# juhyeonkim95/Mitsuba3DopplerToF

Measured on AMD Instinct MI355X. Metric: Mpaths/s (whole node), Doppler Cornell 512x512 64spp, higher is better.
Workload: dtype f32

## Files before the change

### include/dtof.h

```cpp
#ifndef DTOF_H
#define DTOF_H
#include <stdint.h>
#include <stddef.h>

#ifdef __cplusplus
extern "C" {
#endif

#define DTOF_OK            0
#define DTOF_ERR_INVALID   1
#define DTOF_ERR_HIP       2
#define DTOF_ERR_CANCELLED 3

typedef struct dtof_scene   dtof_scene;
typedef struct dtof_sampler dtof_sampler;

const char *dtof_version(void);
const char *dtof_last_error(void);

int dtof_scene_load_file(const char *path, const char *const *param_names, const char *const *param_values,
                         int n_params, dtof_scene **out);
int dtof_scene_load_string(const char *xml, const char *const *param_names, const char *const *param_values,
                           int n_params, dtof_scene **out);
void dtof_scene_destroy(dtof_scene *scene);
// ... 147 lines not shown
int  dtof_sampler_seed(dtof_sampler *s, uint32_t seed, uint32_t wavefront_size);
int  dtof_sampler_set_samples_per_wavefront(dtof_sampler *s, uint32_t spw);
int  dtof_sampler_advance(dtof_sampler *s);
int  dtof_sampler_next_1d(dtof_sampler *s, float *out);
int  dtof_sampler_next_2d(dtof_sampler *s, float *out_xy);
int  dtof_sampler_next_1d_correlate(dtof_sampler *s, const uint8_t *correlate, int correlate_all, float *out);
int  dtof_sampler_next_2d_correlate(dtof_sampler *s, const uint8_t *correlate, int correlate_all, float *out_xy);
int  dtof_sampler_next_1d_time(dtof_sampler *s, int strategy, float antithetic_shift, int stratify_each_interval, float *out);
int  dtof_sampler_get_state(dtof_sampler *s, uint32_t *out7);
int  dtof_sampler_fork(const dtof_sampler *s, dtof_sampler **out);
int  dtof_sampler_clone(const dtof_sampler *s, dtof_sampler **out);
int  dtof_sampler_set_sample_count(dtof_sampler *s, uint32_t sample_count);
int  dtof_sampler_seeded(const dtof_sampler *s);
uint32_t dtof_sampler_wavefront_size(const dtof_sampler *s);
uint32_t dtof_sampler_sample_count(const dtof_sampler *s);

int dtof_eval_modulation(dtof_scene *scene, int mode, const float *t, const float *len, float *out, uint32_t n);

int dtof_ray_intersect(dtof_scene *scene, uint32_t n, const float *rays8, float *out19, int32_t *ids3);
int dtof_ray_intersect_uv(dtof_scene *scene, uint32_t n, const float *rays8, float *out19, int32_t *ids3, float *uv4);
int dtof_ray_test(dtof_scene *scene, uint32_t n, const float *rays8, int32_t *occluded);
int dtof_flat_query(dtof_scene *scene, int form, int any, uint32_t n, const float *rays8, float *out3, int32_t *ids);
int dtof_flat_query_pairs(dtof_scene *scene, int any, uint32_t n, const float *rays8, float *out3, int32_t *ids);
int dtof_tree_query(dtof_scene *scene, int form, int any, uint32_t n, const float *rays8, float *out3, int32_t *ids3);

#define DTOF_COMP_MICROFACET_EVAL          0
#define DTOF_COMP_MICROFACET_PDF           1
#define DTOF_COMP_MICROFACET_G1            2
#define DTOF_COMP_MICROFACET_SAMPLE        3
#define DTOF_COMP_FRESNEL                  4
#define DTOF_COMP_FRESNEL_CONDUCTOR        5
#define DTOF_COMP_RFILTER                  6
#define DTOF_COMP_WARP_COSINE_HEMISPHERE   7
#define DTOF_COMP_WARP_DISK_CONCENTRIC     8
#define DTOF_COMP_WARP_UNIFORM_TRIANGLE    9
#define DTOF_COMP_WARP_UNIFORM_SPHERE     10
#define DTOF_COMP_COORDINATE_SYSTEM       11
#define DTOF_COMP_TEA_FLOAT32             12
#define DTOF_COMP_MATH                    13
int dtof_eval_component(int component, const float *params, int n_params, const float *in, int in_stride, float *out, int out_stride, uint32_t n);

#ifdef __cplusplus
}
#endif
#endif
```

### mitsuba3dopplertof_amd/__init__.py

```python
import ctypes as C
import os

import numpy as np

__all__ = ["load_file", "load_string", "load_dict", "Scene", "Integrator", "Sampler", "DtofError", "render",
           "render_multi_pass", "to_tof_image", "lib_path", "ETimeSampling", "velocity_map_variants", "MOMENT_PLANES", "aov_channels", "AOV_TYPES"]

_HERE = os.path.dirname(os.path.abspath(__file__))
_LIB = None


class DtofError(RuntimeError):
    pass


class ETimeSampling:
    UNIFORM, STRATIFIED, ANTITHETIC, ANTITHETIC_MIRROR, PERIODIC, REGULAR = 0, 1, 2, 3, 4, 5


class _Stats(C.Structure):
    _fields_ = [("n_paths", C.c_uint64), ("n_bounces", C.c_uint64), ("n_shadow_rays", C.c_uint64),
                ("ms_total", C.c_double), ("ms_generate", C.c_double), ("ms_trace", C.c_double),
                ("ms_shade", C.c_double), ("ms_shadow", C.c_double), ("ms_splat", C.c_double),
                ("n_launches_trace", C.c_uint32), ("n_launches_shade", C.c_uint32), ("n_launches_shadow", C.c_uint32),
# ... 98 lines not shown
    L.dtof_eval_component.argtypes = [C.c_int, vp, C.c_int, vp, C.c_int, vp, C.c_int, C.c_uint32]
    L.dtof_render_rows_async.argtypes = [vp, C.c_uint32, C.c_uint32, C.c_int32, C.c_int32, vp, C.c_int, vp]
    L.dtof_clear_async.argtypes = [vp, vp, C.c_size_t]
    L.dtof_camera_rays.argtypes = [vp, C.c_uint32, vp, vp]
    L.dtof_bsdf_eval.argtypes = [vp, C.c_uint32, C.c_uint32, vp, vp]
    L.dtof_bsdf_eval_ex.argtypes = [vp, C.c_uint32, C.c_int, C.c_uint32, vp, vp]
    L.dtof_scene_set_stream.argtypes = [vp, vp]
    L.dtof_scene_set_film_layout.argtypes = [vp, C.c_int32, C.c_uint64]
    L.dtof_render_stripes_async.argtypes = [vp, C.c_uint32, C.c_uint32, C.c_int32, C.c_int32, C.c_int32, vp, C.c_int, vp]
    L.dtof_develop_async.argtypes = [vp, vp, vp, C.c_int64]
    L.dtof_async_collect.argtypes = [vp, vp, vp, C.c_uint32, vp]
    L.dtof_ray_intersect.argtypes = [vp, C.c_uint32, vp, vp, vp]
    L.dtof_ray_intersect_uv.argtypes = [vp, C.c_uint32, vp, vp, vp, vp]
    L.dtof_ray_test.argtypes = [vp, C.c_uint32, vp, vp]
    rows, stripes = [vp, C.c_uint32, C.c_uint32, C.c_int32, C.c_int32, vp, C.c_int, vp], [vp, C.c_uint32, C.c_uint32, C.c_int32, C.c_int32, C.c_int32, vp, C.c_int, vp]
    for name, args in (("dtof_render_variants", [vp, C.c_uint32, C.c_uint32, vp, C.c_int, vp, C.POINTER(_Stats)]),
                       ("dtof_render_rows_variants", rows + [C.POINTER(_Stats)]), ("dtof_render_rows_variants_async", rows),
                       ("dtof_render_stripes_variants", stripes + [C.POINTER(_Stats)]), ("dtof_render_stripes_variants_async", stripes),
                       ("dtof_sample_lanes_variants", [vp, C.c_uint32, C.c_uint32, vp, C.c_int, C.c_uint64, C.c_uint64, vp, vp, vp]),
                       ("dtof_emitter_eval", [vp, C.c_int, C.c_int, C.c_int32, C.c_uint32, vp, vp]),
                       ("dtof_flat_query", [vp, C.c_int, C.c_int, C.c_uint32, vp, vp, vp]),
                       ("dtof_flat_query_pairs", [vp, C.c_int, C.c_uint32, vp, vp, vp]),
                       ("dtof_tree_query", [vp, C.c_int, C.c_int, C.c_uint32, vp, vp, vp]),
                       ("dtof_develop_accumulate_async", [vp, vp, C.c_int32, C.c_uint64, vp, C.c_int64, C.c_int]),
                       ("dtof_velocity_map_async", [vp, vp, C.c_int, vp, vp, C.c_uint32, C.c_double, C.c_double, C.c_int64, vp, vp, vp]),
                       ("dtof_velocity_map_variants", [vp, C.c_int, vp]),
                       ("dtof_render_velocity_map", [vp, C.c_uint32, C.c_uint32, vp, C.c_int, C.c_double, C.c_double, vp, vp, vp, C.POINTER(_Stats)]),
                       ("dtof_render_velocity_map_f64", [vp, C.c_uint32, C.c_uint32, vp, C.c_int, C.c_double, C.c_double, vp, vp, vp, C.POINTER(_Stats)]),
                       ("dtof_render_variants_f64", [vp, C.c_uint32, C.c_uint32, vp, C.c_int, vp, vp, C.POINTER(_Stats)]),
                       ("dtof_render_rows_variants_f64", rows[:-1] + [vp, C.c_int32, C.c_uint64, C.POINTER(_Stats)]),
                       ("dtof_develop_f64_async", [vp, vp, vp, C.c_int64]), ("dtof_develop_rgba_f64_async", [vp, vp, vp, vp, C.c_int64]),
                       ("dtof_moment_planes", [C.c_int]),
                       ("dtof_render_moments", [vp, C.c_uint32, C.c_uint32, C.c_uint32, vp, C.c_int, C.c_int, vp, C.POINTER(_Stats)]),
                       ("dtof_aov_parse", [C.c_char_p, vp, C.c_int, C.POINTER(C.c_int), vp, C.c_size_t, C.POINTER(C.c_int)]),
                       ("dtof_scene_get_aovs", [vp, vp, C.c_size_t]),
                       ("dtof_render_aovs", [vp, C.c_uint32, C.c_uint32, C.c_uint32, vp, C.c_int, C.c_int, vp, C.POINTER(_Stats)]),
                       ("dtof_sample_aov_lanes", [vp, C.c_uint32, C.c_uint32, vp, C.c_int, C.c_uint64, C.c_uint64, vp, vp])):
        if hasattr(L, name):
            getattr(L, name).argtypes = args
    _LIB = L
    return L


FLAT_GEOMETRY = np.array([[1, 0, 0,  0, 1, 0,  0, 0, 1,  1, 0, 0,  0, 1, 0,  0, 0, 1]], np.float32)


# ... 443 lines not shown
                "wi": out[:, 16:19], "ids": ids, "uv": uv[:, 0:2], "prim_uv": uv[:, 2:4], "prim_index": ids[:, 2], "valid": ids[:, 0] >= 0}

    def ray_test(self, o, d, time=0.0, maxt=None):
        rays = self._rays(o, d, time, maxt)
        occ = np.zeros(len(rays), np.int32)
        _check(_lib().dtof_ray_test(self._h, len(rays), rays.ctypes.data, occ.ctypes.data))
        return occ != 0

    FLAT_FORMS = {"generic": 0, "one_wall": 1, "shape": 2}

    def flat_query(self, rays8, form=0, any=False):
        rays = np.ascontiguousarray(rays8, np.float32).reshape(-1, 8)
        form = self.FLAT_FORMS.get(form, form)
        out, ids = np.zeros((len(rays), 3), np.float32), np.zeros(len(rays), np.int32)
        _check(_lib().dtof_flat_query(self._h, int(form), 1 if any else 0, len(rays), rays.ctypes.data, None if any else out.ctypes.data, ids.ctypes.data))
        return ids if any else {"t": out[:, 0], "u": out[:, 1], "v": out[:, 2], "obj": ids}

    def flat_query_pairs(self, rays8, any=False):
        rays = np.ascontiguousarray(rays8, np.float32).reshape(-1, 8)
        out, ids = np.zeros((len(rays), 3), np.float32), np.zeros(len(rays), np.int32)
        _check(_lib().dtof_flat_query_pairs(self._h, 1 if any else 0, len(rays), rays.ctypes.data, None if any else out.ctypes.data, ids.ctypes.data))
        return ids if any else {"t": out[:, 0], "u": out[:, 1], "v": out[:, 2], "obj": ids}

    TREE_FORMS = {"float": 0, "half_overflow": 1, "half_overflow_tlas_lds": 2, "defer_pair": 3, "half_every_shape": 4}

    def tree_query(self, rays8, form=0, any=False):
        rays = np.ascontiguousarray(rays8, np.float32).reshape(-1, 8)
        form = self.TREE_FORMS.get(form, form)
        out, ids = np.zeros((len(rays), 3), np.float32), np.zeros(len(rays) if any else (len(rays), 3), np.int32)
        _check(_lib().dtof_tree_query(self._h, int(form), 1 if any else 0, len(rays), rays.ctypes.data, None if any else out.ctypes.data, ids.ctypes.data))
        return ids if any else {"t": out[:, 0], "u": out[:, 1], "v": out[:, 2], "ids": ids}

    def cancel(self):
        _lib().dtof_cancel(self._h)


COMPONENTS = {"microfacet_eval": (0, 1), "microfacet_pdf": (1, 1), "microfacet_g1": (2, 1), "microfacet_sample": (3, 4), "fresnel": (4, 4),
              "fresnel_conductor": (5, 1), "rfilter": (6, 1), "warp_cosine_hemisphere": (7, 3), "warp_disk_concentric": (8, 2),
              "warp_uniform_triangle": (9, 2), "warp_uniform_sphere": (10, 3), "coordinate_system": (11, 6), "tea_float32": (12, 1), "math": (13, 1)}


def eval_component(name, inputs, params=()):
    comp, n_out = COMPONENTS[name]
    x = np.ascontiguousarray(np.atleast_2d(np.asarray(inputs, np.float32)))
    p = np.ascontiguousarray(np.asarray(params, np.float32).reshape(-1))
    out = np.zeros((len(x), n_out), np.float32)
# ... 183 lines not shown
```

### mitsuba3dopplertof_amd/csrc/dtof_kernels.h

```cpp
#pragma once
#include <stdint.h>
#include <hip/hip_runtime.h>
#include "dtof_math.h"

namespace dtof {

constexpr uint32_t kChunkBlocks = 8;
constexpr uint32_t kMaxInline = 4;
constexpr int kMaxOffsets = 4;

struct RenderParams {
    float s2c[16];
    float cam_to_world[12];
    float near_clip, far_clip, shutter_open, shutter_open_time;
    int32_t orthographic;
    float aperture_radius, focus_distance;
    int32_t crop_x, crop_y, crop_w, crop_h;
    float scale_x, scale_y, offset_x, offset_y;
    int32_t filter; float filter_radius, inv_radius;
    float gauss_coeff[10];
    float filter_b, filter_c;
    uint32_t base_seed, seed, seed_value;
    uint32_t spp, spp_log2;
    uint32_t tcn, pcn;
// ... 149 lines not shown
constexpr uint32_t kHeadlineC2Facts = (DTOF_HEADLINE_C2) != 0 && kHeadlineFusedFacts != 0 ? (kHeadlineFusedFacts | (DTOF_HEADLINE_C2)) : 0u;
static_assert(((DTOF_HEADLINE_C2) & ~kFactsSampling) == 0, "DTOF_HEADLINE_C2 names route facts only (bits 13 and up)");
#ifndef DTOF_HEADLINE_SHAPE_COUNT
#define DTOF_HEADLINE_SHAPE_COUNT 5
#endif
#ifndef DTOF_HEADLINE_SHAPE_WALL
#define DTOF_HEADLINE_SHAPE_WALL 2
#endif
constexpr uint32_t kHeadlineShapeFacts = (DTOF_HEADLINE_SHAPE_COUNT) != 0 && (kHeadlineC2Facts & kFactOneWall) != 0 ? (kHeadlineC2Facts | flat_shape_fact(DTOF_HEADLINE_SHAPE_COUNT, DTOF_HEADLINE_SHAPE_WALL)) : 0u;
static_assert((DTOF_HEADLINE_SHAPE_COUNT) == 0 || (kHeadlineC2Facts & kFactOneWall) == 0 || (kHeadlineShapeFacts & kFactFlatShape) != 0, "a shape has 1 .. 8 objects and the wall among them");
#ifndef DTOF_HEADLINE_PAIR
#define DTOF_HEADLINE_PAIR 1
#endif
#ifndef DTOF_STREAM_JUMPS
#define DTOF_STREAM_JUMPS 1
#endif
#ifndef DTOF_PAIR_SAMPLES
#define DTOF_PAIR_SAMPLES 1
#endif
constexpr uint32_t kHeadlinePairFacts = DTOF_HEADLINE_PAIR && kHeadlineShapeFacts != 0 ? (kHeadlineShapeFacts | kFactPairSamples) : 0u;
#ifndef DTOF_PAIR_WALK_PRIMARY
#define DTOF_PAIR_WALK_PRIMARY 1
#endif
#ifdef DTOF_TRAVERSAL_STATS
constexpr bool kPairWalkCompiled = false;
#else
constexpr bool kPairWalkCompiled = true;
#endif
constexpr bool pair_walk_shape(uint32_t facts) { return (facts & kFactOneWall) != 0 && flat_shape_count(facts) == 5 && flat_shape_wall(facts) == 2; }
#ifndef DTOF_FLAT_SHAPE_ANY
#define DTOF_FLAT_SHAPE_ANY 1
#endif
#ifndef DTOF_FLAT_SHAPE_CLOSEST
#define DTOF_FLAT_SHAPE_CLOSEST 1
#endif
#ifndef DTOF_WALL_FRAMES
#define DTOF_WALL_FRAMES 1
#endif
#ifndef DTOF_RESIDENT_FACTS
#define DTOF_RESIDENT_FACTS 0x37f
#endif
constexpr uint32_t kResidentFacts = DTOF_RESIDENT_FACTS;

struct ShadeLaunch { bool staged; int mode; uint32_t waves, grid, lds, lds_flat; hipStream_t stream; ShadeArgs args; uint32_t facts; };
uint32_t launch_shade_plain(bool area, bool k4, const ShadeLaunch &L);
void launch_shade_mesh(bool area, bool k4, const ShadeLaunch &L);
// ... 77 lines not shown
```

### mitsuba3dopplertof_amd/csrc/dtof_render.hip

```cpp
#include "../../include/dtof.h"
#include "dtof_kernels.h"
#include "dtof_reconstruct.h"
#include "dtof_film64.h"
#include "dtof_moments.h"
#include "dtof_aov.h"
#include "dtof_flat_query.h"
#include "dtof_tree_query.h"
#include "dtof_scene.h"
#include "dtof_math.h"
#include <atomic>
#include <dlfcn.h>
#include <cstdio>
#include <cstring>
#include <cstdlib>
#include <cmath>
#include <string>
#include <memory>
#include <vector>

using namespace dtof;

namespace {

thread_local std::string g_last_error;

struct HipError : std::runtime_error { using std::runtime_error::runtime_error; };
#define HIP_CHECK(expr) do { hipError_t e_ = (expr); if (e_ != hipSuccess) \
    throw HipError(std::string(#expr) + ": " + hipGetErrorString(e_)); } while (0)

// ... 1800 lines not shown
        if (n & 1u) throw std::runtime_error("dtof_flat_query_pairs: an odd number of rays");
        if (n > (1u << 24)) throw std::runtime_error("dtof_flat_query_pairs: more than 2^24 rays in one call");
        for (uint32_t i = 0; i < n; i += 2) {
            const float *a = rays8 + (size_t) i * 8, *b = a + 8;
            if (memcmp(a, b, 24) != 0 || memcmp(a + 7, b + 7, 4) != 0)
                throw std::runtime_error("dtof_flat_query_pairs: rays " + std::to_string(i) + " and " + std::to_string(i + 1) + " differ in o, d or maxt");
        }
        const SceneTraits t = scene_traits(*sc);
        const FlatChoice c = flat_choice(t, t.blas_triangles <= 32768 && sc->host.textures.empty(), true, true);
        if (!kFlatQueryPairsBuilt || c.flat_objects == 0 || !(c.facts & kFactOneWall) || (c.facts & kFlatShapeFields) != (flat_query_facts(2) & kFlatShapeFields))
            throw std::runtime_error("dtof_flat_query_pairs: the pair form is compiled for a flat table of 5 rectangles whose one instance, of one rectangle, is at index 2" +
                                     (c.flat_objects ? ", this table has " + std::to_string(c.flat_objects) + " objects" : std::string(", this scene has no flat table")));
        ensure_device(sc);
        DevBuf<float> dr, dout; DevBuf<int32_t> dids;
        dr.ensure((size_t) n * 8); dout.ensure(any ? 1 : (size_t) n * 3); dids.ensure(n);
        if (n) HIP_CHECK(hipMemcpy(dr.p, rays8, (size_t) n * 32, hipMemcpyHostToDevice));
        launch_flat_query(sc->d_blob.p, (uint32_t) sc->blob.size(), t.flat_off, c.flat_objects, c.memo_obj, kFlatQueryPairs, any != 0, dr.p, dout.p, dids.p, n, nullptr);
        HIP_CHECK(hipGetLastError());
        if (n && !any) HIP_CHECK(hipMemcpy(out3, dout.p, (size_t) n * 12, hipMemcpyDeviceToHost));
        if (n) HIP_CHECK(hipMemcpy(ids, dids.p, (size_t) n * 4, hipMemcpyDeviceToHost));
    });
}

int dtof_tree_query(dtof_scene *sc, int form, int any, uint32_t n, const float *rays8, float *out3, int32_t *ids3) {
    return guarded([&] {
        if (!sc || (n && (!rays8 || !ids3 || (!any && !out3)))) throw std::runtime_error("null argument");
        if (n > (1u << 24)) throw std::runtime_error("dtof_tree_query: more than 2^24 rays in one call");
        const SceneTraits t = scene_traits(*sc);
        const TreeQueryScene q { t.stack_depth, t.n_tlas_nodes, t.has_nodes16, t.has_analytic };
        if (const char *why = tree_query_refusal(form, q)) throw std::runtime_error(std::string("dtof_tree_query: ") + why);
        ensure_device(sc);
        const size_t per = any ? 1 : 3;
        DevBuf<float> dr, dout; DevBuf<int32_t> dids;
        dr.ensure((size_t) n * 8); dout.ensure(any ? 1 : (size_t) n * 3); dids.ensure((size_t) n * per);
        if (n) HIP_CHECK(hipMemcpy(dr.p, rays8, (size_t) n * 32, hipMemcpyHostToDevice));
        launch_tree_query(sc->d_blob.p, q, form, any != 0, dr.p, dout.p, dids.p, n, nullptr);
        HIP_CHECK(hipGetLastError());
        if (n && !any) HIP_CHECK(hipMemcpy(out3, dout.p, (size_t) n * 12, hipMemcpyDeviceToHost));
        if (n) HIP_CHECK(hipMemcpy(ids3, dids.p, (size_t) n * per * 4, hipMemcpyDeviceToHost));
    });
}

#ifdef DTOF_TRAVERSAL_STATS
int dtof_debug_traversal_stats_n(unsigned long long *out8, uint32_t n) {
    return guarded([&] {
        HIP_CHECK(hipDeviceSynchronize());
// ... 10 lines not shown
```

### mitsuba3dopplertof_amd/csrc/dtof_sampling.h

```cpp
#pragma once
#include "dtof_kernels.h"
#include "dtof_scene.h"
#include "dtof_math.h"

#ifndef DTOF_D
#define DTOF_D __device__ __forceinline__
#endif

namespace dtof {

struct Rng { uint64_t state, inc; };
DTOF_D float next_f32(Rng &r) { return pcg_next_f32(r.state, r.inc); }
DTOF_D Rng seed_stream(uint32_t seed_value, uint32_t index) {
    uint32_t v0, v1; tea32(seed_value, index, v0, v1);
    Rng r; pcg_seed(v0, v1, r.state, r.inc); return r;
}
DTOF_D uint64_t stream_inc(uint32_t seed_value, uint32_t index) {
    uint32_t v0, v1; tea32(seed_value, index, v0, v1);
    return ((uint64_t) v1 << 1) | 1u;
}
DTOF_D float next_correlate(Rng &main, Rng &path, bool correlate) {
    uint64_t old = correlate ? path.state : main.state;
    path.state = path.state * kPcgMult + path.inc;
    main.state = main.state * kPcgMult + main.inc;
// ... 89 lines not shown
    V3 near_p = mk(r0 * iw, r1 * iw, r2 * iw);
    if (!PERSPECTIVE_ONLY && rp.orthographic) {
        o = xf_point(rp.cam_to_world, near_p);
        dw = normalize(xf_vector(rp.cam_to_world, mk(0.f, 0.f, 1.f)));
        maxt = rp.far_clip - rp.near_clip;
        return;
    }
    const bool lens = !PERSPECTIVE_ONLY && rp.aperture_radius != 0.f;
    V3 d;
    if (lens) {
        float tx, ty; concentric_disk(apx, apy, tx, ty);
        const V3 aperture_p = mk(rp.aperture_radius * tx, rp.aperture_radius * ty, 0.f);
        const float f_dist = rp.focus_distance / near_p.z;
        d = normalize(near_p * f_dist - aperture_p);
        o = xf_point(rp.cam_to_world, aperture_p);
    } else {
        d = normalize(near_p);
        o = mk(rp.cam_to_world[3], rp.cam_to_world[7], rp.cam_to_world[11]);
    }
    dw = xf_vector(rp.cam_to_world, d);
    float inv_z = rcp(d.z), near_t = rp.near_clip * inv_z, far_t = rp.far_clip * inv_z;
    o = o + dw * near_t;
    maxt = far_t - near_t;
}

template <bool PERSPECTIVE_ONLY = false, uint32_t FACTS = 0>
DTOF_D PrimaryLane generate_lane(const RenderParams &rp, uint32_t lane, bool wave_pixel = false, uint32_t vlane = 0) {
    constexpr bool F_SINGLE_PASS = (FACTS & kFactSinglePass) != 0, F_DOPPLER_CORR = (FACTS & kFactDopplerCorr) != 0, F_CORRELATED = (FACTS & kFactCorrelated) != 0;
    constexpr bool F_STRAT = (FACTS & kFactStratifiedPairs) != 0 && F_DOPPLER_CORR, F_SHIFTS = facts_lane_shifts(FACTS);
    const bool needs_tm = !F_STRAT && (F_DOPPLER_CORR || (rp.integrator == 0 && rp.sampler_kind == SAMPLER_CORRELATED)) && rp.time_sampling >= TIME_ANTITHETIC;
    Rng main, tm, path; tm.state = 0; tm.inc = 1;
    uint2 *const carried = !F_SINGLE_PASS && rp.n_passes > 1 ? rp.pass_rng + (size_t) (vlane - rp.pass_first) * 3 : nullptr;
    const uint32_t pass = F_SINGLE_PASS ? 0u : rp.pass;
    if (pass == 0 && wave_pixel && needs_tm && rp.tcn == 2 && rp.pcn == 2) {
        main = seed_stream(rp.seed_value, lane);
        const bool odd = lane & 1u;
        uint32_t a0, a1; tea32(rp.seed_value + (odd ? 2u : 1u), lane >> 1, a0, a1);
        const uint32_t b0 = (uint32_t) __builtin_amdgcn_update_dpp(0, (int) a0, 0xb1, 0xf, 0xf, false), b1 = (uint32_t) __builtin_amdgcn_update_dpp(0, (int) a1, 0xb1, 0xf, 0xf, false);
        pcg_seed(odd ? b0 : a0, odd ? b1 : a1, tm.state, tm.inc);
        pcg_seed(odd ? a0 : b0, odd ? a1 : b1, path.state, path.inc);
    } else if (pass == 0) {
        main = seed_stream(rp.seed_value, lane);
        if (needs_tm) tm = seed_stream(rp.seed_value + 1, fdiv(lane, rp.d_tcn));
        path = seed_stream(rp.seed_value + 2, F_STRAT ? lane >> 1 : fdiv(lane, rp.d_pcn));
    } else {
        const uint2 a = carried[0], b = carried[1], c = carried[2];
// ... 46 lines not shown
```

### mitsuba3dopplertof_amd/csrc/dtof_shade.h

```cpp
#pragma once
#include "dtof_device.h"
#include <atomic>
#include <initializer_list>
#include <type_traits>

namespace dtof {


DTOF_D uint32_t wave_append(bool pred, uint32_t &running) {
    const uint64_t mask = __ballot(pred);
    const uint32_t slot = running + (uint32_t) __popcll(mask & ((1ull << __lane_id()) - 1ull));
    running += (uint32_t) __popcll(mask);
    return slot;
}

struct BsdfOut { V3 val, weight, wo; float pdf, bs_pdf, bs_eta; bool bs_delta, bs_null; };
template <int SPEC, bool HAVE_WO = false>
DTOF_D void bsdf_eval_pdf_sample(const SceneView &sv, const DShape *sh, Surface &si, V3 wo, bool active_em, float sample_1, float s2x, float s2y, BsdfOut &out, bool want_sample = true, const V3 *diffuse_wo = nullptr) {
    const bool masked = SPEC && (sh->flags & SF_MASK);
    bool null_pick = false; float opacity = 1.f;
    if (masked) { opacity = mask_opacity_at(sv, sh, si.u, si.v); null_pick = !(sample_1 < opacity); sample_1 = sample_1 / opacity; }
    const bool blend = SPEC == 2 && (sh->flags & SF_BLEND);
    float blend_w = 0.f; bool pick_1 = false;
    if (blend) {
// ... 280 lines not shown
template <bool AREA, bool MESH, int SPEC, bool ONE_EMITTER = false>
void launch_emitter_eval_level(const uint8_t *scene, int mode, uint32_t index, float pmf, const float *in, float *out, uint32_t n, hipStream_t s) {
    if (n) hipLaunchKernelGGL((k_emitter_eval<AREA, MESH, SPEC, ONE_EMITTER>), dim3(nblk(n)), dim3(kBlock), 0, s, scene, mode, index, pmf, in, out, n);
}

template <bool LDS, int MODE, bool AREA, int KMAX, bool MESH, int SPEC, int RESW = 0, bool RH16 = false, uint32_t FACTS = 0>
#ifndef DTOF_MESH_WAVES
#define DTOF_MESH_WAVES 3
#endif
#ifndef DTOF_K4_RES_LDS
#define DTOF_K4_RES_LDS 1
#endif
__global__ __launch_bounds__(RESW ? RESW * 64 : kShadeBlock, RESW ? RESW / 4 : (MODE == 2 && !MESH && !SPEC && KMAX == 1) ? 4 : (MODE != 0 && MESH) ? ((SPEC && KMAX > 1) ? 2 : DTOF_MESH_WAVES) : 1) void k_shade(ShadeArgs args_by_value) {
    constexpr bool FUSED = MODE != 0, FIRST = MODE == 2;
    static_assert(FACTS == 0 || MODE == 2, "plan facts describe a first-bounce launch");
    constexpr bool F_SINGLE_PASS = (FACTS & kFactSinglePass) != 0, F_DOPPLER_CORR = (FACTS & kFactDopplerCorr) != 0, F_NO_LANE_OUT = (FACTS & kFactNoLaneOutput) != 0;
    constexpr bool F_IDENTITY = (FACTS & kFactIdentityQueue) != 0, F_NO_RR = (FACTS & kFactNoRoulette) != 0, F_CORRELATED = (FACTS & kFactCorrelated) != 0;
    constexpr bool F_WHOLE_PATH = (FACTS & kFactWholePath) != 0, F_ONE_BLOCK = (FACTS & kFactOneBlock) != 0, F_ONE_EMITTER = (FACTS & kFactOneEmitter) != 0;
    constexpr bool F_WAVE_PIXEL = (FACTS & kFactWavePixel) != 0;
    constexpr bool F_FLAT = (FACTS & kFactFlat) != 0, F_ONE_WALL = (FACTS & kFactOneWall) != 0, F_FUSED_SPLAT = (FACTS & kFactFusedSplat) != 0;
    constexpr bool F_EMITTER_SAMPLED = (FACTS & kFactEmitterSampled) != 0, F_ID24 = (FACTS & kFactIdShift24) != 0, F_SHIFTS = facts_lane_shifts(FACTS);
    constexpr bool F_PAIR = (FACTS & kFactPairSamples) != 0, JUMPS = F_PAIR && DTOF_STREAM_JUMPS, PAIR = F_PAIR && DTOF_PAIR_SAMPLES;
    constexpr bool WALK_PRIMARY = F_PAIR && DTOF_PAIR_WALK_PRIMARY && pair_walk_shape(FACTS);
    static_assert(!F_PAIR || F_WAVE_PIXEL, "a lane reads its partner's registers: the whole wave is active where it does");
    static_assert(!F_PAIR || (!AREA && SPEC == 0 && KMAX == 1 && F_ONE_EMITTER), "a diffuse BSDF picks no lobe and a lone point light samples nothing: of an iteration's six draws only s2x and s2y are read");
    static_assert(!F_PAIR || (F_NO_RR && F_CORRELATED && F_DOPPLER_CORR && F_WHOLE_PATH && F_SINGLE_PASS && (FACTS & kFactStratifiedPairs) != 0), "every draw comes from the stream lanes 2k and 2k + 1 share, none is looked at for roulette, no state outlives the launch");
    constexpr bool F_FRAMES = F_ONE_WALL && DTOF_WALL_FRAMES;
    static_assert(!F_FLAT || (!MESH && SPEC == 0 && RESW == 0), "trace_flat serves the staged rectangle-only diffuse kernels");
    static_assert(!F_ONE_WALL || F_FLAT, "the one wall is an object of the flat table");
    static_assert(!F_FUSED_SPLAT || KMAX == 1, "the fused splat is the one-film kernels'");
    static_assert(!F_WAVE_PIXEL || F_IDENTITY, "whole waves of one pixel are provable for an identity queue only");
    static_assert(!F_ONE_BLOCK || RESW == 0, "blocks per segment belong to the classic launch");
    constexpr bool RES_LDS = RESW != 0 && KMAX > 1 && DTOF_K4_RES_LDS;
    constexpr bool S16 = RESW != 0 && KMAX > 1;
    static_assert(!RES_LDS || 3 * KMAX == (int) kParkWords + 1, "the film-state columns hold all but the last float of the K results");
    constexpr bool PARK_ST = DTOF_PARK && RESW == 16 && KMAX == 1;
    constexpr bool PARK = DTOF_PARK && RESW == 16 && (KMAX == 1 || RES_LDS);
    constexpr uint32_t kRngAt = RES_LDS ? kParkWords : 0u;
    constexpr int KREG = RES_LDS ? 1 : KMAX;
    constexpr uint32_t kStackStride = RESW ? RESW * 64 : kShadeBlock;
    static_assert(RESW == 0 || (MODE == 2 && !LDS && MESH), "the resident stage exists for the unstaged fused first-bounce kernel with mesh code");
    static_assert(!RH16 || RESW != 0, "half-float LDS planes belong to the resident stage");
    extern __shared__ uint4 lds[];
    __shared__ uint32_t s_inline_all[(RESW ? RESW : 1) * 2 * kMaxInline];
    typedef const char __attribute__((address_space(4))) *KernargBytes;
    const KernargBytes kernarg = (KernargBytes) __builtin_amdgcn_kernarg_segment_ptr();
// ... 37 lines not shown
        sv_res.isect = (const DTriIsect *) (small + gh->off_isect);
        sv_res.emitters = (const DEmitter *) (small + gh->off_emitters);
    }
    for (;;) {
    uint32_t seg, sub_index = 0;
    if (RESW) {
        uint32_t taken = 0;
        if (lane_id == 0) taken = atomicAdd(A0.q.seg_counter, 1u);
        uint32_t unit = (uint32_t) __builtin_amdgcn_readfirstlane((int) taken);
        if (unit >= A0.n_seg * sub) break;
        unit = A0.n_seg * sub - 1u - unit;
        seg = sub > 1 ? unit / sub : unit; sub_index = sub > 1 ? unit - seg * sub : 0u;
    } else {
        seg = sub > 1 ? blockIdx.x / sub : blockIdx.x; sub_index = sub > 1 ? blockIdx.x - seg * sub : 0u;
    }
    const uint32_t count = seg_count(F_IDENTITY ? nullptr : A0.count_in, seg, A0.rp.n_lanes);
    uint32_t n_alive = 0, n_shadow = 0;
    if (FIRST && lane_id < 2 * kMaxInline) s_inline[lane_id] = 0;
    if (count != 0) {
    const uint8_t *base = LDS ? stage_scene(A0.scene, A0.scene_bytes, lds) : A0.scene;
    SceneView sv = RESW ? sv_res : make_view(base);
    if (FUSED) { sv.memo_obj = A0.rp.memo_obj; sv.memo = (float *) (lds + stage_words) + (RESW ? wave_id * kMemoWords * kMemoStride + lane_id : threadIdx.x); sv.memo_m = memo_m_lds; }
    const bool have_memo = F_ONE_WALL || (FUSED && sv.memo_obj != 0xffffffffu);
    for (uint32_t cbase = sub > 1 ? sub_index * unit_lanes : 0u; cbase < (sub > 1 ? (sub_index + 1) * unit_lanes < count ? (sub_index + 1) * unit_lanes : count : count); cbase += kShadeBlock) {
    uint32_t rebase = 0;
    asm volatile("" : "+s"(rebase));
    const ShadeArgs &A = *(const ShadeArgs *) (kernarg + rebase);
    const RenderParams &rp = A.rp; const Queues &q = A.q;
    const uint32_t *const qin = F_IDENTITY ? nullptr : A.qin; uint32_t *const qout = A.qout; const uint32_t depth0 = A.depth, trace_next_last = F_WHOLE_PATH ? 0u : A.trace_next;
    LaneDebug *const dbg = F_NO_LANE_OUT ? nullptr : A.dbg;
    const uint32_t flat = FUSED && !MESH ? rp.flat_objects : 0u;
    uint32_t j = cbase + lane_id;
    bool in_range = F_WAVE_PIXEL || j < count;
    bool alive = false, want_shadow = false;
    uint32_t l = 0;
    float4 sha = make_float4(0.f, 0.f, 0.f, 0.f), shb = sha, nra = sha, nrb = sha; float3 cand[KREG];
#pragma unroll
    for (int k = 0; k < KREG; ++k) cand[k] = make_float3(0.f, 0.f, 0.f);
    float3 rbase[KREG];
#pragma unroll
    for (int k = 0; k < KREG; ++k) rbase[k] = make_float3(0.f, 0.f, 0.f);
    V3 pend_thr = mk(0, 0, 0), pend_v = mk(0, 0, 0); float pend_len = 0.f;
    float *const park = RES_LDS || PARK ? (float *) (lds + stage_words) + memo_words + A0.res_park_off + threadIdx.x : nullptr;
    float res_last = 0.f;
    auto res_get = [&](int k) -> float4 {
        if (RES_LDS) return make_float4(park[(3 * k) * kStackStride], park[(3 * k + 1) * kStackStride], 3 * k + 2 < (int) kParkWords ? park[(3 * k + 2) * kStackStride] : res_last, 0.f);
// ... 31 lines not shown
    const bool valid_start = SPEC && rp.has_env && !rp.hide_emitters;
    bool valid_reg = valid_start;
    float memo_m[12], memo_inv[12];
    typename std::conditional<F_FRAMES, WallFrames, NoFrames>::type wf;
    if constexpr (F_FRAMES) {
        wf.n = mk(0.f, 0.f, 1.f); wf.s = mk(1.f, 0.f, 0.f);
        wf.table = (const DFlatFrame *) ((const uint4 *) ((const DFlatObject *) (sv.base + rp.flat_off) + rp.flat_objects) + 1 + rp.flat_objects);
    }
    V3 pair_wo = mk(0.f, 0.f, 1.f), pair_wo_next = pair_wo;
    bool lane_on = in_range;
#ifdef DTOF_TRAVERSAL_STATS
    constexpr uint64_t kPoisonState = 0xdeadbeefcafef00dull;
    if (!in_range) { main.state = path.state = kPoisonState; const float pz = u2f(0x7fc0dead); ra = rb = st = make_float4(pz, pz, pz, pz); }
#define DTOF_POISON_CHECK() do { if (main.state == kPoisonState || path.state == kPoisonState || f2u(st.x) == 0x7fc0deadu || f2u(ra.x) == 0x7fc0deadu) DTOF_STAT(14); } while (0)
#else
#define DTOF_POISON_CHECK() ((void) 0)
#endif
    const bool wave_pixel = F_WAVE_PIXEL || (FIRST && rp.spp_log2 != 0xffffffffu && rp.spp_log2 >= 6 && (rp.lane_base & 63u) == 0 && count - cbase >= (uint32_t) kShadeBlock);
    const bool fuse_splat = F_FUSED_SPLAT || (FIRST && A.film != nullptr);
    float2 pos_reg = make_float2(0.f, 0.f);
    if (in_range) {
        l = qin ? qin[seg * kSeg + j] : seg * kSeg + j;
        if (FIRST) {
            const PrimaryLane pl = generate_lane<SPEC == 0, FACTS>(rp, global_lane<FACTS>(rp, rp.lane_base + l), wave_pixel, rp.lane_base + l);
            ra = pl.ray_a; rb = pl.ray_b; main = pl.main; path = pl.path; st = make_float4(1.f, 1.f, 1.f, 0.f);
            if constexpr (PAIR) {
                const bool odd = lane_id & 1u;
                uint64_t sx;
                if constexpr (JUMPS) {
                    constexpr uint64_t m3 = pcg_pow(3), g3 = pcg_geom(3), m9 = pcg_pow(9), g9 = pcg_geom(9);
                    sx = path.state * (odd ? m9 : m3) + path.inc * (odd ? g9 : g3);
                } else {
                    uint64_t s3 = path.state;
                    for (int i = 0; i < 3; ++i) s3 = s3 * kPcgMult + path.inc;
                    uint64_t s9 = s3;
                    for (int i = 0; i < 6; ++i) s9 = s9 * kPcgMult + path.inc;
                    sx = odd ? s9 : s3;
                }
                const uint64_t sy = sx * kPcgMult + path.inc;
                const V3 mine = cosine_hemisphere(pcg_output_f32(sx), pcg_output_f32(sy));
                pair_wo = mk(__int_as_float(__builtin_amdgcn_update_dpp(0, __float_as_int(mine.x), 0xa0, 0xf, 0xf, false)),
                             __int_as_float(__builtin_amdgcn_update_dpp(0, __float_as_int(mine.y), 0xa0, 0xf, 0xf, false)),
                             __int_as_float(__builtin_amdgcn_update_dpp(0, __float_as_int(mine.z), 0xa0, 0xf, 0xf, false)));
                pair_wo_next = mk(__int_as_float(__builtin_amdgcn_update_dpp(0, __float_as_int(mine.x), 0xf5, 0xf, 0xf, false)),
                                  __int_as_float(__builtin_amdgcn_update_dpp(0, __float_as_int(mine.y), 0xf5, 0xf, 0xf, false)),
                                  __int_as_float(__builtin_amdgcn_update_dpp(0, __float_as_int(mine.z), 0xf5, 0xf, 0xf, false)));
            }
// ... 397 lines not shown
```

Before: 19150.

## Share paired camera-ray setup across lane pairs via chunked pair generation

For the pair-sample headline kernel, primary lane generation is split into a per-pair part (camera jitter, camera ray, path stream) and a per-lane part (main stream, time sample). Each lane of a chunk computes one pair part, either for the current chunk or for the next chunk. The result is carried in registers across two consecutive 64-lane chunks and delivered to partner lanes with ds_bpermute or DPP. This removes redundant camera-ray computation, since lanes 2k and 2k+1 share the same ray, at the cost of carrying twelve extra registers through the loop and adding cross-lane moves. A standalone test entry point is also added to validate the lane setup.

```diff
diff --git a/include/dtof.h b/include/dtof.h
--- a/include/dtof.h
+++ b/include/dtof.h
@@ -193,6 +193,7 @@
 int dtof_ray_test(dtof_scene *scene, uint32_t n, const float *rays8, int32_t *occluded);
 int dtof_flat_query(dtof_scene *scene, int form, int any, uint32_t n, const float *rays8, float *out3, int32_t *ids);
 int dtof_flat_query_pairs(dtof_scene *scene, int any, uint32_t n, const float *rays8, float *out3, int32_t *ids);
+int dtof_pair_setup_lanes(dtof_scene *scene, int form, uint32_t seed, uint32_t spp, uint64_t lane_begin, uint64_t n, uint32_t *out16);
 int dtof_tree_query(dtof_scene *scene, int form, int any, uint32_t n, const float *rays8, float *out3, int32_t *ids3);
 
 #define DTOF_COMP_MICROFACET_EVAL          0
diff --git a/mitsuba3dopplertof_amd/__init__.py b/mitsuba3dopplertof_amd/__init__.py
--- a/mitsuba3dopplertof_amd/__init__.py
+++ b/mitsuba3dopplertof_amd/__init__.py
@@ -144,6 +144,7 @@
                        ("dtof_flat_query", [vp, C.c_int, C.c_int, C.c_uint32, vp, vp, vp]),
                        ("dtof_flat_query_pairs", [vp, C.c_int, C.c_uint32, vp, vp, vp]),
                        ("dtof_tree_query", [vp, C.c_int, C.c_int, C.c_uint32, vp, vp, vp]),
+                       ("dtof_pair_setup_lanes", [vp, C.c_int, C.c_uint32, C.c_uint32, C.c_uint64, C.c_uint64, vp]),
                        ("dtof_develop_accumulate_async", [vp, vp, C.c_int32, C.c_uint64, vp, C.c_int64, C.c_int]),
                        ("dtof_velocity_map_async", [vp, vp, C.c_int, vp, vp, C.c_uint32, C.c_double, C.c_double, C.c_int64, vp, vp, vp]),
                        ("dtof_velocity_map_variants", [vp, C.c_int, vp]),
@@ -633,6 +634,11 @@
         _check(_lib().dtof_flat_query_pairs(self._h, 1 if any else 0, len(rays), rays.ctypes.data, None if any else out.ctypes.data, ids.ctypes.data))
         return ids if any else {"t": out[:, 0], "u": out[:, 1], "v": out[:, 2], "obj": ids}
 
+    def pair_setup_lanes(self, seed, spp, lane_begin, n, form=1):
+        out = np.zeros((int(n), 16), np.uint32)
+        _check(_lib().dtof_pair_setup_lanes(self._h, int(form), seed, spp, lane_begin, n, out.ctypes.data))
+        return out
+
     TREE_FORMS = {"float": 0, "half_overflow": 1, "half_overflow_tlas_lds": 2, "defer_pair": 3, "half_every_shape": 4}
 
     def tree_query(self, rays8, form=0, any=False):
diff --git a/mitsuba3dopplertof_amd/csrc/dtof_kernels.h b/mitsuba3dopplertof_amd/csrc/dtof_kernels.h
--- a/mitsuba3dopplertof_amd/csrc/dtof_kernels.h
+++ b/mitsuba3dopplertof_amd/csrc/dtof_kernels.h
@@ -195,6 +195,14 @@
 #ifndef DTOF_PAIR_WALK_PRIMARY
 #define DTOF_PAIR_WALK_PRIMARY 1
 #endif
+#ifndef DTOF_PAIR_SETUP
+#define DTOF_PAIR_SETUP 1
+#endif
+#ifndef DTOF_PAIR_SETUP_BPERMUTE
+#define DTOF_PAIR_SETUP_BPERMUTE 1
+#endif
+constexpr uint32_t kFactsLaneSplit = kFactSinglePass | kFactDopplerCorr | kFactCorrelated | kFactStratifiedPairs | kFactWavePixel;
+constexpr bool lane_split_facts(uint32_t facts) { return (facts & kFactsLaneSplit) == kFactsLaneSplit; }
 #ifdef DTOF_TRAVERSAL_STATS
 constexpr bool kPairWalkCompiled = false;
 #else
diff --git a/mitsuba3dopplertof_amd/csrc/dtof_pair_setup.h b/mitsuba3dopplertof_amd/csrc/dtof_pair_setup.h
--- /dev/null
+++ b/mitsuba3dopplertof_amd/csrc/dtof_pair_setup.h
@@ -0,0 +1,63 @@
+#pragma once
+#include "dtof_kernels.h"
+#include "dtof_sampling.h"
+
+namespace dtof {
+
+constexpr uint32_t kPairSetupLaneFacts = kFactsLaneSplit | kFactPow2Strata;
+static_assert(kHeadlinePairFacts == 0 || (kHeadlinePairFacts & kPairSetupLaneFacts) == kPairSetupLaneFacts, "the headline kernel generates its lanes under these facts");
+constexpr uint32_t kPairChunk = 64;
+constexpr uint32_t kPairSetupWords = 16;
+void launch_pair_setup_lanes(const RenderParams &rp, int form, uint32_t *out, hipStream_t s);
+
+constexpr uint32_t kPairPartWords = 12;
+DTOF_D PairPart pair_part_zero() {
+    PairPart p; p.o = mk(0.f, 0.f, 0.f); p.d = mk(0.f, 0.f, 1.f); p.maxt = 0.f; p.pos = make_float2(0.f, 0.f); p.path_state = 0ull; p.path_sel = 0u;
+    return p;
+}
+DTOF_D void pair_part_words(const PairPart &c, uint32_t (&w)[kPairPartWords]) {
+    w[0] = f2u(c.o.x); w[1] = f2u(c.o.y); w[2] = f2u(c.o.z); w[3] = f2u(c.d.x); w[4] = f2u(c.d.y); w[5] = f2u(c.d.z); w[6] = f2u(c.maxt); w[7] = f2u(c.pos.x); w[8] = f2u(c.pos.y);
+    w[9] = (uint32_t) c.path_state; w[10] = (uint32_t) (c.path_state >> 32); w[11] = c.path_sel;
+}
+DTOF_D PairPart pair_part_of_words(const uint32_t (&r)[kPairPartWords]) {
+    PairPart p;
+    p.o = mk(u2f(r[0]), u2f(r[1]), u2f(r[2])); p.d = mk(u2f(r[3]), u2f(r[4]), u2f(r[5])); p.maxt = u2f(r[6]); p.pos = make_float2(u2f(r[7]), u2f(r[8]));
+    p.path_state = (uint64_t) r[9] | ((uint64_t) r[10] << 32); p.path_sel = r[11];
+    return p;
+}
+template <bool ODD>
+DTOF_D PairPart pair_fetch_dpp(const PairPart &c) {
+    uint32_t w[kPairPartWords], r[kPairPartWords];
+    pair_part_words(c, w);
+#pragma unroll
+    for (uint32_t i = 0; i < kPairPartWords; ++i) r[i] = (uint32_t) __builtin_amdgcn_update_dpp(0, (int) w[i], ODD ? 0xf5 : 0xa0, 0xf, 0xf, false);
+    return pair_part_of_words(r);
+}
+DTOF_D PairPart pair_fetch_bpermute(const PairPart &c, uint32_t lane_id, bool odd) {
+    uint32_t w[kPairPartWords], r[kPairPartWords];
+    pair_part_words(c, w);
+    const int addr = (int) (((lane_id & ~1u) | (odd ? 1u : 0u)) << 2);
+#pragma unroll
+    for (uint32_t i = 0; i < kPairPartWords; ++i) r[i] = (uint32_t) __builtin_amdgcn_ds_bpermute(addr, (int) w[i]);
+    return pair_part_of_words(r);
+}
+template <uint32_t FACTS, bool BPERMUTE = DTOF_PAIR_SETUP_BPERMUTE != 0>
+DTOF_D PrimaryLane pair_setup_chunk(const RenderParams &rp, uint32_t first, uint32_t lane_id, bool second, PairPart &carried) {
+    const PixelInfo here = pixel_info<true>(rp, first >> rp.spp_log2);
+    if (!second) {
+        const PixelInfo next = pixel_info<true>(rp, (first + kPairChunk) >> rp.spp_log2);
+        const bool odd = lane_id & 1u;
+        carried = generate_pair_part<FACTS>(rp, first + (odd ? kPairChunk : 0u) + lane_id, odd ? next.posx : here.posx, odd ? next.posy : here.posy);
+    }
+    PairPart pp;
+    if (BPERMUTE) pp = pair_fetch_bpermute(carried, lane_id, second);
+    else if (second) pp = pair_fetch_dpp<true>(carried); else pp = pair_fetch_dpp<false>(carried);
+    const LanePart lp = generate_lane_part<FACTS>(rp, first + lane_id, here.perm_seed);
+    PrimaryLane pl;
+    pl.ray_a = make_float4(pp.o.x, pp.o.y, pp.o.z, lp.time);
+    pl.ray_b = make_float4(pp.d.x, pp.d.y, pp.d.z, pp.maxt);
+    pl.main = lp.main; pl.path.state = pp.path_state; pl.path.inc = ((uint64_t) pp.path_sel << 1) | 1u; pl.pos = pp.pos;
+    return pl;
+}
+
+}
diff --git a/mitsuba3dopplertof_amd/csrc/dtof_pair_setup.hip b/mitsuba3dopplertof_amd/csrc/dtof_pair_setup.hip
--- /dev/null
+++ b/mitsuba3dopplertof_amd/csrc/dtof_pair_setup.hip
@@ -0,0 +1,32 @@
+#include "dtof_device.h"
+#include "dtof_pair_setup.h"
+
+namespace dtof {
+
+template <int FORM>
+__global__ __launch_bounds__(kShadeBlock) void k_pair_setup_lanes(RenderParams rp, uint32_t *out) {
+    constexpr uint32_t FACTS = kPairSetupLaneFacts;
+    const uint32_t seg = blockIdx.x, lane_id = threadIdx.x;
+    const uint32_t count = seg_count(nullptr, seg, rp.n_lanes);
+    PairPart carried = pair_part_zero();
+    for (uint32_t cbase = 0; cbase < count; cbase += kShadeBlock) {
+        const uint32_t l = seg * kSeg + cbase + lane_id;
+        PrimaryLane pl;
+        if (FORM == 1) pl = pair_setup_chunk<FACTS>(rp, rp.lane_base + seg * kSeg + cbase, lane_id, ((cbase >> 6) & 1u) != 0, carried);
+        else pl = generate_lane<true, FACTS>(rp, global_lane<FACTS>(rp, rp.lane_base + l), true, rp.lane_base + l);
+        uint4 *const w = (uint4 *) (out + (size_t) l * kPairSetupWords);
+        w[0] = make_uint4(f2u(pl.pos.x), f2u(pl.pos.y), f2u(pl.ray_a.w), f2u(pl.ray_a.x));
+        w[1] = make_uint4(f2u(pl.ray_a.y), f2u(pl.ray_a.z), f2u(pl.ray_b.x), f2u(pl.ray_b.y));
+        w[2] = make_uint4(f2u(pl.ray_b.z), f2u(pl.ray_b.w), (uint32_t) pl.path.state, (uint32_t) (pl.path.state >> 32));
+        w[3] = make_uint4((uint32_t) (pl.path.inc >> 1), 0u, 0u, 0u);
+    }
+}
+
+void launch_pair_setup_lanes(const RenderParams &rp, int form, uint32_t *out, hipStream_t s) {
+    if (!rp.n_lanes) return;
+    const uint32_t grid = nseg(rp.n_lanes);
+    if (form == 1) hipLaunchKernelGGL((k_pair_setup_lanes<1>), dim3(grid), dim3(kShadeBlock), 0, s, rp, out);
+    else hipLaunchKernelGGL((k_pair_setup_lanes<0>), dim3(grid), dim3(kShadeBlock), 0, s, rp, out);
+}
+
+}
diff --git a/mitsuba3dopplertof_amd/csrc/dtof_render.hip b/mitsuba3dopplertof_amd/csrc/dtof_render.hip
--- a/mitsuba3dopplertof_amd/csrc/dtof_render.hip
+++ b/mitsuba3dopplertof_amd/csrc/dtof_render.hip
@@ -5,6 +5,7 @@
 #include "dtof_moments.h"
 #include "dtof_aov.h"
 #include "dtof_flat_query.h"
+#include "dtof_pair_setup.h"
 #include "dtof_tree_query.h"
 #include "dtof_scene.h"
 #include "dtof_math.h"
@@ -1851,6 +1852,37 @@
     });
 }
 
+int dtof_pair_setup_lanes(dtof_scene *sc, int form, uint32_t seed, uint32_t spp, uint64_t lane_begin, uint64_t n, uint32_t *out16) {
+    return guarded([&] {
+        if (!sc || (n && !out16)) throw std::runtime_error("null argument");
+        if (form != 0 && form != 1) throw std::runtime_error("dtof_pair_setup_lanes: form must be 0 (per lane) or 1 (chunk pairs)");
+        if (!sc->host.has_sensor) throw std::runtime_error("the scene does not contain a sensor");
+        if ((lane_begin & 63u) != 0 || (n & 63u) != 0) throw std::runtime_error("dtof_pair_setup_lanes: lane_begin and n must be multiples of 64 (whole chunks)");
+        if (n > (1u << 24)) throw std::runtime_error("dtof_pair_setup_lanes: more than 2^24 lanes in one call");
+        FramePlan p; RenderRequest rq; rq.seed = seed; rq.spp = spp;
+        plan_lanes(p, sc, rq);
+        RenderParams &rp = p.rp;
+        const auto need = [](bool ok, const char *what) { if (!ok) throw std::runtime_error(std::string("dtof_pair_setup_lanes: lane generation is compiled for ") + what); };
+        need(p.n_passes == 1, "a single pass");
+        need(rp.integrator == 0 && rp.sampler_kind == SAMPLER_CORRELATED, "the dopplertofpath integrator with the correlated sampler");
+        need(rp.path_correlation_depth > 0, "a path-correlated camera sample (path_correlation_depth > 0)");
+        need(rp.time_sampling == TIME_STRATIFIED && rp.stratify != 0 && rp.tcn == 2 && rp.pcn == 2 && rp.shutter_open_time > 0.f && rp.spp > 1,
+             "stratified time sampling per interval with pairs (time_correlate_number = path_correlate_number = 2) and an open shutter");
+        need(rp.n_stratum >= 2 && (rp.n_stratum & (rp.n_stratum - 1u)) == 0, "a power-of-two stratum count");
+        need(rp.spp_log2 != 0xffffffffu && rp.spp_log2 >= 6, "a power-of-two sample count of at least 64 (whole waves of one pixel)");
+        need(!rp.orthographic && rp.aperture_radius == 0.f, "the perspective camera");
+        const uint64_t total = (uint64_t) sc->host.sensor.crop_w * sc->host.sensor.crop_h * rp.spp;
+        if (lane_begin + n > total) throw std::runtime_error("lane range exceeds the wavefront");
+        if (n == 0) return;
+        ensure_device(sc);
+        rp.lane_base = (uint32_t) lane_begin; rp.n_lanes = (uint32_t) n;
+        DevBuf<uint32_t> dout; dout.ensure((size_t) n * kPairSetupWords);
+        launch_pair_setup_lanes(rp, form, dout.p, nullptr);
+        HIP_CHECK(hipGetLastError());
+        HIP_CHECK(hipMemcpy(out16, dout.p, (size_t) n * kPairSetupWords * 4, hipMemcpyDeviceToHost));
+    });
+}
+
 int dtof_tree_query(dtof_scene *sc, int form, int any, uint32_t n, const float *rays8, float *out3, int32_t *ids3) {
     return guarded([&] {
         if (!sc || (n && (!rays8 || !ids3 || (!any && !out3)))) throw std::runtime_error("null argument");
diff --git a/mitsuba3dopplertof_amd/csrc/dtof_sampling.h b/mitsuba3dopplertof_amd/csrc/dtof_sampling.h
--- a/mitsuba3dopplertof_amd/csrc/dtof_sampling.h
+++ b/mitsuba3dopplertof_amd/csrc/dtof_sampling.h
@@ -135,6 +135,36 @@
     float inv_z = rcp(d.z), near_t = rp.near_clip * inv_z, far_t = rp.far_clip * inv_z;
     o = o + dw * near_t;
     maxt = far_t - near_t;
+}
+
+struct PairPart { V3 o, d; float maxt; float2 pos; uint64_t path_state; uint32_t path_sel; };
+template <uint32_t FACTS>
+DTOF_D PairPart generate_pair_part(const RenderParams &rp, uint32_t lane, float posx, float posy) {
+    static_assert(lane_split_facts(FACTS), "the pair's piece is the text of generate_lane under these facts");
+    Rng path = seed_stream(rp.seed_value + 2, lane >> 1);
+    const uint64_t sx = path.state, sy = sx * kPcgMult + path.inc;
+    path.state = sy * kPcgMult + path.inc;
+    const float jx = pcg_output_f32(sx), jy = pcg_output_f32(sy);
+    const float spx = posx + jx, spy = posy + jy;
+    const float ax = fmaf(spx, rp.scale_x, rp.offset_x), ay = fmaf(spy, rp.scale_y, rp.offset_y);
+    PairPart pp;
+    camera_ray<true>(rp, ax, ay, .5f, .5f, pp.o, pp.d, pp.maxt);
+    pp.pos = make_float2(spx, spy); pp.path_state = path.state; pp.path_sel = (uint32_t) (path.inc >> 1);
+    return pp;
+}
+struct LanePart { Rng main; float time; };
+template <uint32_t FACTS>
+DTOF_D LanePart generate_lane_part(const RenderParams &rp, uint32_t lane, uint32_t perm_seed) {
+    static_assert(lane_split_facts(FACTS), "the lane's piece is the text of generate_lane under these facts");
+    LanePart lp; Rng tm; tm.state = 0; tm.inc = 1;
+    lp.main = seed_stream(rp.seed_value, lane);
+    lp.main.state = lp.main.state * kPcgMult + lp.main.inc;
+    lp.main.state = lp.main.state * kPcgMult + lp.main.inc;
+    uint32_t dim = 0;
+    const float u = next_time<FACTS>(rp, lp.main, tm, lane & (rp.spp - 1u), perm_seed, dim);
+    const float time = rp.shutter_open + u * rp.shutter_open_time;
+    lp.time = time < rp.T ? time : time - rp.T;
+    return lp;
 }
 
 template <bool PERSPECTIVE_ONLY = false, uint32_t FACTS = 0>
diff --git a/mitsuba3dopplertof_amd/csrc/dtof_shade.h b/mitsuba3dopplertof_amd/csrc/dtof_shade.h
--- a/mitsuba3dopplertof_amd/csrc/dtof_shade.h
+++ b/mitsuba3dopplertof_amd/csrc/dtof_shade.h
@@ -1,5 +1,6 @@
 #pragma once
 #include "dtof_device.h"
+#include "dtof_pair_setup.h"
 #include <atomic>
 #include <initializer_list>
 #include <type_traits>
@@ -326,6 +327,8 @@
     constexpr bool F_EMITTER_SAMPLED = (FACTS & kFactEmitterSampled) != 0, F_ID24 = (FACTS & kFactIdShift24) != 0, F_SHIFTS = facts_lane_shifts(FACTS);
     constexpr bool F_PAIR = (FACTS & kFactPairSamples) != 0, JUMPS = F_PAIR && DTOF_STREAM_JUMPS, PAIR = F_PAIR && DTOF_PAIR_SAMPLES;
     constexpr bool WALK_PRIMARY = F_PAIR && DTOF_PAIR_WALK_PRIMARY && pair_walk_shape(FACTS);
+    constexpr bool PAIR_SETUP = F_PAIR && DTOF_PAIR_SETUP && F_ONE_BLOCK && F_IDENTITY && SPEC == 0 && lane_split_facts(FACTS);
+    static_assert(kPairChunk == (uint32_t) kShadeBlock, "a chunk of the pair setup is one block of k_shade");
     static_assert(!F_PAIR || F_WAVE_PIXEL, "a lane reads its partner's registers: the whole wave is active where it does");
     static_assert(!F_PAIR || (!AREA && SPEC == 0 && KMAX == 1 && F_ONE_EMITTER), "a diffuse BSDF picks no lobe and a lone point light samples nothing: of an iteration's six draws only s2x and s2y are read");
     static_assert(!F_PAIR || (F_NO_RR && F_CORRELATED && F_DOPPLER_CORR && F_WHOLE_PATH && F_SINGLE_PASS && (FACTS & kFactStratifiedPairs) != 0), "every draw comes from the stream lanes 2k and 2k + 1 share, none is looked at for roulette, no state outlives the launch");
@@ -409,6 +412,7 @@
     SceneView sv = RESW ? sv_res : make_view(base);
     if (FUSED) { sv.memo_obj = A0.rp.memo_obj; sv.memo = (float *) (lds + stage_words) + (RESW ? wave_id * kMemoWords * kMemoStride + lane_id : threadIdx.x); sv.memo_m = memo_m_lds; }
     const bool have_memo = F_ONE_WALL || (FUSED && sv.memo_obj != 0xffffffffu);
+    PairPart pair_carried = pair_part_zero();
     for (uint32_t cbase = sub > 1 ? sub_index * unit_lanes : 0u; cbase < (sub > 1 ? (sub_index + 1) * unit_lanes < count ? (sub_index + 1) * unit_lanes : count : count); cbase += kShadeBlock) {
     uint32_t rebase = 0;
     asm volatile("" : "+s"(rebase));
@@ -486,7 +490,9 @@
     if (in_range) {
         l = qin ? qin[seg * kSeg + j] : seg * kSeg + j;
         if (FIRST) {
-            const PrimaryLane pl = generate_lane<SPEC == 0, FACTS>(rp, global_lane<FACTS>(rp, rp.lane_base + l), wave_pixel, rp.lane_base + l);
+            PrimaryLane pl;
+            if constexpr (PAIR_SETUP) pl = pair_setup_chunk<FACTS, DTOF_PAIR_SETUP_BPERMUTE != 0>(rp, rp.lane_base + seg * kSeg + cbase, lane_id, ((cbase >> 6) & 1u) != 0, pair_carried);
+            else pl = generate_lane<SPEC == 0, FACTS>(rp, global_lane<FACTS>(rp, rp.lane_base + l), wave_pixel, rp.lane_base + l);
             ra = pl.ray_a; rb = pl.ray_b; main = pl.main; path = pl.path; st = make_float4(1.f, 1.f, 1.f, 0.f);
             if constexpr (PAIR) {
                 const bool odd = lane_id & 1u;
```

After: 19350 (median of 6 runs). 1.01x the previous value.
